# edwinyosorahardjo/compressjs-flattened

Hardware: AMD Instinct MI355X
Metric: bzip2 -9 compress MB/s at 1/2/4/8 MI355X; bit-exact output size vs ref (higher is better)
Workload: dtype u32; 1 GPU; Bzip2.compressFile level 9 (899981-byte blocks) on 1 x 100000000 bytes enwik8-shaped synthetic text (tools/textgen.c seed 1), device-resident; per_gpu_bytes=100000000, level=9, parallelism=1 GPU

## Files before the change

### compressjs-flattened_amd/csrc/ctx.h

```cpp
#pragma once
#include "cjs_internal.h"
#include "rle1.h"
#include "mtf.h"
#include "huff.h"

namespace cjs {
struct BatchWork;
void batch_destroy(BatchWork* b);
struct BatchDelete { void operator()(BatchWork* b) const { batch_destroy(b); } };
}

struct cjs_ctx {
  int device = 0, level = 0;
  uint32_t cap = 0;
  size_t max_input = 0, max_blocks = 0, range_blocks = 0;
  cjs::Arena arena;
  cjs::Rle1Work rle;
  cjs::BwtWork bwt;
  cjs::MtfWork mtf;
  cjs::HuffWork huff;
  uint8_t* d_blocks = nullptr;
  uint8_t* d_U = nullptr;
  uint32_t* d_pidx = nullptr;
  cjs::Owner<cjs::BatchWork*, cjs::BatchDelete> batch;
  cjs::Pinned<uint64_t> h_scalars;
  cjs::Stream stream;
  cjs::Stream side;
  cjs::Event ev_join, ev_fork;
  cjs::Stream tail;
  cjs::Event ev_tail, ev_piece[8];
  cjs::EventTimer timer;
  uint32_t sh_nb = 0, sh_first = 0, sh_cnt = 0, sh_state = 0;
  bool stage_times = true;
};

namespace cjs {
int blocks_through_tables(cjs_ctx* c, const uint8_t* d_in, size_t n, uint32_t nb, uint32_t last_len, uint32_t f, uint32_t cnt, cjs_stats* st, bool stage_times);
}
```

### compressjs-flattened_amd/csrc/mtf.h

```cpp
#pragma once
#include "cjs_internal.h"

namespace cjs {

struct MtfBufs {
  uint32_t* hpos;
  uint8_t* hsym;
  uint8_t* hrank;
  uint8_t* lists;
  uint16_t* A;
  uint32_t* freq;
  uint8_t* alist;
  uint32_t *asz, *nheads, *npos;
  int* segkeys;
  size_t seg_stride;
  size_t list_stride, a_stride, hstride;
};

struct MtfWork {
  size_t max_blocks = 0;
  uint32_t stride = 0;
  MtfBufs b{};
  static size_t list_stride_for(uint32_t stride) { return ((size_t)(stride + 255) / 256 + 1) * 256; }
  static size_t seg_stride_for(uint32_t stride) { return ((size_t)stride + 8191) / 8192 + 1; }
  static size_t hstride_for(uint32_t stride) { return ((size_t)stride + 15) & ~(size_t)15; }
  static size_t a_stride_for(uint32_t stride) { return ((size_t)stride + 2 + 7) & ~(size_t)7; }
  static size_t bytes_needed(size_t max_blocks, uint32_t stride);
  int carve(Arena& a, size_t max_blocks, uint32_t stride);
  MtfWork view(size_t first, size_t count) const {
    MtfWork v = *this;
    v.max_blocks = count;
    v.b.hpos += first * b.hstride; v.b.hsym += first * b.hstride; v.b.hrank += first * b.hstride;
    v.b.lists += first * b.list_stride; v.b.A += first * b.a_stride; v.b.freq += first * 258; v.b.alist += first * 256;
    v.b.asz += first; v.b.nheads += first; v.b.npos += first;
    v.b.segkeys += first * b.seg_stride * 256;
    return v;
  }
};

int mtf_run(hipStream_t s, MtfWork& w, const uint8_t* d_U, uint32_t nb, const uint32_t* d_blen);

}
```

### compressjs-flattened_amd/csrc/mtf.hip

```cpp
#include "cjs_internal.h"
#include "prims.hpp"
#include "mtf.h"

namespace cjs {

#ifndef CJS_MTF_CHUNK
#define CJS_MTF_CHUNK 512
#endif
#ifndef CJS_MTF_CL_THREADS
#define CJS_MTF_CL_THREADS 256
#endif
constexpr int MTF_CHUNK = CJS_MTF_CHUNK;
constexpr int MTF_CL_THREADS = CJS_MTF_CL_THREADS;

constexpr uint32_t MT_TILE = 4096;
constexpr uint32_t HT_PER = 16, HT_TILE = 1024 * HT_PER;
__device__ __forceinline__ uint32_t head_flags4(const uint8_t* __restrict__ u, bool row0, uint32_t p0, uint32_t n, uint32_t& mine) {
  mine = 0;
  if (p0 >= n) return 0u;
  const uintptr_t a = (uintptr_t)(u + p0);
  const uint32_t* al = reinterpret_cast<const uint32_t*>(a & ~(uintptr_t)3);
  const uint32_t sh = (uint32_t)(a & 3);
  const bool first = row0 && p0 == 0;
  const uint32_t wm = first ? 0u : al[-1], w0 = al[0], w1 = sh ? al[1] : 0u;
  mine = __builtin_amdgcn_alignbyte(w1, w0, sh);
  uint32_t prev = __builtin_amdgcn_alignbyte(w0, wm, sh) >> 24;
  uint32_t fm = 0;
#pragma unroll
  for (int j = 0; j < 4; j++) {
    const uint32_t p = p0 + j, c = (mine >> (8 * j)) & 0xFFu;
    if (p < n && (p == 0 || c != prev)) fm |= 1u << j;
    prev = c;
  }
  return fm;
}
__global__ __launch_bounds__(1024) void mtf_head_count(const uint8_t* __restrict__ U, uint32_t stride, const uint32_t* __restrict__ blen,
                                                       uint32_t* __restrict__ tcnt, uint32_t tpb, uint32_t* __restrict__ uflag) {
  __shared__ uint32_t used[256];
  __shared__ uint32_t sm[16];
  const uint32_t blk = blockIdx.y, tile = blockIdx.x, n = blen[blk];
  const uint32_t base = tile * HT_TILE;
  if (base >= n) { if (threadIdx.x == 0) tcnt[(size_t)blk * tpb + tile] = 0; return; }
  const uint8_t* u = U + (size_t)blk * stride;
  if (threadIdx.x < 256) used[threadIdx.x] = 0;
  __syncthreads();
  const uint32_t p0 = base + threadIdx.x * HT_PER;
  uint32_t m4[4] = {0, 0, 0, 0};
  uint32_t prev = 0, cnt = 0;
  if (p0 < n) {
    const uintptr_t a = (uintptr_t)(u + p0);
    const uint32_t* al = reinterpret_cast<const uint32_t*>(a & ~(uintptr_t)3);
    const uint32_t sh = (uint32_t)(a & 3);
    const bool first = blk == 0 && p0 == 0;
    const uint32_t wm = first ? 0u : al[-1], w0 = al[0], w1 = al[1], w2 = al[2], w3 = al[3], w4 = sh ? al[4] : 0u;
    m4[0] = __builtin_amdgcn_alignbyte(w1, w0, sh); m4[1] = __builtin_amdgcn_alignbyte(w2, w1, sh);
    m4[2] = __builtin_amdgcn_alignbyte(w3, w2, sh); m4[3] = __builtin_amdgcn_alignbyte(w4, w3, sh);
    prev = __builtin_amdgcn_alignbyte(w0, wm, sh) >> 24;
  }
#pragma unroll
  for (int j = 0; j < (int)HT_PER; j++) {
    const uint32_t p = p0 + j;
    const uint32_t c = p < n ? (m4[j >> 2] >> (8 * (j & 3))) & 0xFFu : 0u;
    if (p < n && (p == 0 || c != prev)) { cnt++; used[c] = 1; }
    prev = c;
  }
  const uint32_t tot = block_sum<1024>(cnt, sm);
  if (threadIdx.x == 0) tcnt[(size_t)blk * tpb + tile] = tot;
  if (threadIdx.x < 256 && used[threadIdx.x]) uflag[(size_t)blk * 258 + threadIdx.x] = 1;
}
__global__ __launch_bounds__(1024) void mtf_head_write(const uint8_t* __restrict__ U, uint32_t stride, const uint32_t* __restrict__ blen,
                                                       MtfBufs mb, const uint32_t* __restrict__ tcnt, uint32_t tpb) {
  __shared__ uint32_t sm[16];
  const uint32_t blk = blockIdx.y, tile = blockIdx.x, n = blen[blk];
  const uint32_t base = tile * HT_TILE;
  if (base >= n) return;
  const uint8_t* u = U + (size_t)blk * stride;
  uint32_t* hpos = mb.hpos + (size_t)blk * mb.hstride;
  uint8_t* hsym = mb.hsym + (size_t)blk * mb.hstride;
  uint32_t run = tcnt[(size_t)blk * tpb + tile];
  for (uint32_t r = 0; r < HT_TILE / 4096u; r++) {
    const uint32_t p0 = base + r * 4096u + threadIdx.x * 4u;
    if (base + r * 4096u >= n) break;
    uint32_t mine;
    const uint32_t fm = head_flags4(u, blk == 0, p0, n, mine);
    uint32_t tot;
    uint32_t o = run + block_excl_sum<1024>((uint32_t)__builtin_popcount(fm), sm, tot);
#pragma unroll
    for (int j = 0; j < 4; j++) if ((fm >> j) & 1u) { hpos[o] = p0 + j; hsym[o] = (uint8_t)(mine >> (8 * j)); o++; }
    run += tot;
  }
}
__global__ __launch_bounds__(1024) void mtf_head_scan(MtfBufs mb, uint32_t* __restrict__ tcnt, uint32_t tpb, const uint32_t* __restrict__ uflag) {
  __shared__ uint32_t sm[16];
  const uint32_t blk = blockIdx.x;
  uint32_t tot;
  const uint32_t v = threadIdx.x < tpb ? tcnt[(size_t)blk * tpb + threadIdx.x] : 0u;
  const uint32_t ex = block_excl_sum<1024>(v, sm, tot);
  if (threadIdx.x < tpb) tcnt[(size_t)blk * tpb + threadIdx.x] = ex;
  if (threadIdx.x == 0) mb.nheads[blk] = tot;
  const uint32_t f = threadIdx.x < 256 ? uflag[(size_t)blk * 258 + threadIdx.x] : 0u;
  uint32_t asz;
  const uint32_t ax = block_excl_sum<1024>(f, sm, asz);
  if (f) mb.alist[(size_t)blk * 256 + ax] = (uint8_t)threadIdx.x;
  if (threadIdx.x == 0) mb.asz[blk] = asz;
}

constexpr int MTF_SEG = 32;
__global__ __launch_bounds__(256) void mtf_seg_last(MtfBufs mb) {
  __shared__ int last[4][256];
  const uint32_t blk = blockIdx.y, seg = blockIdx.x, H = mb.nheads[blk];
  const uint32_t h0 = seg * MTF_SEG * MTF_CHUNK;
  if (h0 >= H) return;
  const uint32_t h1 = h0 + MTF_SEG * MTF_CHUNK < H ? h0 + MTF_SEG * MTF_CHUNK : H;
  const uint8_t* hsym = mb.hsym + (size_t)blk * mb.hstride;
#pragma unroll
  for (int r = 0; r < 4; r++) last[r][threadIdx.x] = -1;
  __syncthreads();
  int* mine = last[threadIdx.x & 3];
  for (uint32_t h = h0 + threadIdx.x; h < h1; h += 256) atomicMax(&mine[hsym[h]], (int)h);
  __syncthreads();
  const int a01 = last[0][threadIdx.x] > last[1][threadIdx.x] ? last[0][threadIdx.x] : last[1][threadIdx.x];
  const int a23 = last[2][threadIdx.x] > last[3][threadIdx.x] ? last[2][threadIdx.x] : last[3][threadIdx.x];
  mb.segkeys[((size_t)blk * mb.seg_stride + seg) * 256 + threadIdx.x] = a01 > a23 ? a01 : a23;
}
__global__ __launch_bounds__(256) void mtf_seg_scan(MtfBufs mb) {
  __shared__ uint32_t used[256];
  const uint32_t blk = blockIdx.x, H = mb.nheads[blk], asz = mb.asz[blk];
  const uint32_t nseg = (H + MTF_SEG * MTF_CHUNK - 1) / (MTF_SEG * MTF_CHUNK);
  used[threadIdx.x] = 0;
  __syncthreads();
  if (threadIdx.x < asz) used[mb.alist[(size_t)blk * 256 + threadIdx.x]] = 1;
  __syncthreads();
  const int d = threadIdx.x;
  int key = used[d] ? 255 - d : -1000;
  int* sk = mb.segkeys + (size_t)blk * mb.seg_stride * 256;
  for (uint32_t sgi = 0; sgi < nseg; sgi++) {
    const int l = sk[(size_t)sgi * 256 + d];
    sk[(size_t)sgi * 256 + d] = key;
    if (l >= 0) key = 256 + l;
  }
}
__global__ __launch_bounds__(MTF_CL_THREADS) void mtf_chunk_lists(MtfBufs mb) {
  __shared__ int keys[256];
  __shared__ uint8_t symof[256];
  __shared__ uint8_t uof[256];
  __shared__ uint32_t part[4][256];
  const uint32_t blk = blockIdx.y, seg = blockIdx.x, H = mb.nheads[blk], nu = mb.asz[blk];
  const uint32_t nch = (H + MTF_CHUNK - 1) / MTF_CHUNK;
  const uint32_t c0 = seg * MTF_SEG;
  if (c0 >= nch) return;
  const uint32_t c1 = c0 + MTF_SEG < nch ? c0 + MTF_SEG : nch;
  const uint8_t* hsym = mb.hsym + (size_t)blk * mb.hstride;
  uint8_t* lists = mb.lists + (size_t)blk * mb.list_stride;
  if (threadIdx.x < nu) {
    const uint8_t sym = mb.alist[(size_t)blk * 256 + threadIdx.x];
    symof[threadIdx.x] = sym; uof[sym] = (uint8_t)threadIdx.x;
    keys[threadIdx.x] = mb.segkeys[((size_t)blk * mb.seg_stride + seg) * 256 + sym];
  }
  __syncthreads();
  constexpr uint32_t NQ = MTF_CL_THREADS / 256;
  const uint32_t d = threadIdx.x & 255u, q = threadIdx.x >> 8, per = (nu + NQ - 1u) / NQ;
  const uint32_t j0 = q * per < nu ? q * per : nu, j1 = j0 + per < nu ? j0 + per : nu;
  for (uint32_t c = c0; c < c1; c++) {
    if (d < nu) {
      const int kd = keys[d];
      uint32_t cnt = 0;
      for (uint32_t j = j0; j < j1; j++) cnt += keys[j] > kd;
      part[q][d] = cnt;
    }
    __syncthreads();
    if (threadIdx.x < nu) {
      uint32_t p = 0;
#pragma unroll
      for (uint32_t qq = 0; qq < NQ; qq++) p += part[qq][d];
      lists[(size_t)c * 256 + p] = symof[d];
    }
    __syncthreads();
    for (uint32_t i = threadIdx.x; i < MTF_CHUNK; i += MTF_CL_THREADS) {
      const uint32_t h = c * MTF_CHUNK + i;
      if (h < H) atomicMax(&keys[uof[hsym[h]]], (int)(256 + h));
    }
    __syncthreads();
  }
}

constexpr int LROW = 260;
constexpr int MTF_RW = 16;
constexpr uint32_t MTF_NR = 4 * MTF_RW;
#ifndef CJS_MTF_TIERS
#define CJS_MTF_TIERS 0, 4, 8, 10, 12, 14, 16
#endif
constexpr int MTF_NTIER = 6;
__device__ constexpr int MTF_TIER[MTF_NTIER + 1] = {CJS_MTF_TIERS};
__device__ __forceinline__ uint32_t zero_bytes(uint32_t v) { return (v - 0x01010101u) & ~v & 0x80808080u; }
__device__ __forceinline__ uint32_t umin(uint32_t a, uint32_t b) { return a < b ? a : b; }
__device__ __forceinline__ uint32_t first_bit_or_ones(uint32_t z) {
  uint32_t f;
  asm("v_ffbl_b32 %0, %1" : "=v"(f) : "v"(z));
  return f;
}
template <int K> __device__ __forceinline__ uint32_t spread_bit(uint32_t v) {
  uint32_t f;
  asm("v_bfe_i32 %0, %1, %2, 1" : "=v"(f) : "v"(v), "n"(K));
  return f;
}
template <int K, int K1> __device__ __forceinline__ uint32_t mtf_search_words(const uint32_t (&l)[MTF_RW], uint32_t bc, uint32_t m) {
  if constexpr (K < K1) {
    const uint32_t ka = first_bit_or_ones(zero_bytes(l[K] ^ bc)) | (32u * K);
    const uint32_t kb = first_bit_or_ones(zero_bytes(l[K + 1] ^ bc)) | (32u * (K + 1));
    return mtf_search_words<K + 2, K1>(l, bc, umin(m, umin(ka, kb)));
  } else {
    return m;
  }
}
template <int T> __device__ __forceinline__ uint32_t mtf_search_tier(const uint32_t (&l)[MTF_RW], uint32_t bc, uint32_t m) {
  return mtf_search_words<MTF_TIER[T], MTF_TIER[T + 1]>(l, bc, m);
}
template <int K, int K0> __device__ __forceinline__ void mtf_shift_words(uint32_t (&l)[MTF_RW], uint32_t bc, uint32_t above, uint32_t g1, uint32_t pm) {
  if constexpr (K >= K0) {
    const uint32_t g = spread_bit<K>(above);
    const uint32_t sh = __builtin_amdgcn_alignbyte(l[K], K ? l[K ? K - 1 : 0] : bc, 3);
    const uint32_t mk = ~g1 | (~g & pm);
    l[K] = (sh & mk) | (l[K] & ~mk);
    mtf_shift_words<K - 1, K0>(l, bc, above, g, pm);
  }
}
template <int T> __device__ __forceinline__ void mtf_shift_tier(uint32_t (&l)[MTF_RW], uint32_t bc, uint32_t above, uint32_t pm) {
  mtf_shift_words<MTF_TIER[T + 1] - 1, MTF_TIER[T]>(l, bc, above, spread_bit<MTF_TIER[T + 1]>(above), pm);
}
__global__ __launch_bounds__(256) void mtf_replay(uint32_t stride, MtfBufs mb) {
  __shared__ uint8_t L[256 * LROW];
  const uint32_t blk = blockIdx.y, H = mb.nheads[blk], asz = mb.asz[blk];
  const uint32_t nch = (H + MTF_CHUNK - 1) / MTF_CHUNK;
  const uint32_t c = blockIdx.x * 256 + threadIdx.x;
  if (blockIdx.x * 256 >= nch) return;
  if (c >= nch) return;
  const uint8_t* hsym = mb.hsym + (size_t)blk * mb.hstride;
  uint8_t* hrank = mb.hrank + (size_t)blk * mb.hstride;
  const uint8_t* lst = mb.lists + (size_t)blk * mb.list_stride + (size_t)c * 256;
  uint8_t* my = L + threadIdx.x * LROW;
  uint32_t l[MTF_RW];
#pragma unroll
  for (int k = 0; k < MTF_RW; k += 4) {
    const uint4 f = *reinterpret_cast<const uint4*>(lst + 4 * k);
    l[k] = f.x; l[k + 1] = f.y; l[k + 2] = f.z; l[k + 3] = f.w;
  }
  for (uint32_t j = MTF_NR; j < asz; j++) my[j] = lst[j];
  const uint32_t h0 = c * MTF_CHUNK, h1 = h0 + MTF_CHUNK < H ? h0 + MTF_CHUNK : H;
  uint4 sv_next = *reinterpret_cast<const uint4*>(hsym + h0);
  for (uint32_t hb = h0; hb < h1; hb += 16) {
    const uint4 sv = sv_next;
    if (hb + 16 < h1) sv_next = *reinterpret_cast<const uint4*>(hsym + hb + 16);
    uint32_t sw[4] = {sv.x, sv.y, sv.z, sv.w}, rw[4] = {0, 0, 0, 0};
    if (hb + 16 > h1) {
      const uint32_t nv = h1 - hb;
#pragma unroll
      for (int q = 1; q < 16; q++)
        if ((uint32_t)q >= nv) {
          const uint32_t p = (sw[(q - 1) >> 2] >> (8 * ((q - 1) & 3))) & 0xFFu;
          sw[q >> 2] = (sw[q >> 2] & ~(0xFFu << (8 * (q & 3)))) | (p << (8 * (q & 3)));
        }
    }
#pragma unroll
    for (int q = 0; q < 16; q++) {
      const uint32_t bc = __builtin_amdgcn_perm(0u, sw[q >> 2], 0x01010101u * (uint32_t)(q & 3));
      uint32_t m = mtf_search_tier<0>(l, bc, ~0u);
      int tier = 0;
      bool more = __any(m == ~0u);
      if (more) { m = mtf_search_tier<1>(l, bc, m); tier = 1; more = __any(m == ~0u); }
      if (more) { m = mtf_search_tier<2>(l, bc, m); tier = 2; more = __any(m == ~0u); }
      if (more) { m = mtf_search_tier<3>(l, bc, m); tier = 3; more = __any(m == ~0u); }
      if (more) { m = mtf_search_tier<4>(l, bc, m); tier = 4; more = __any(m == ~0u); }
      if (more) { m = mtf_search_tier<5>(l, bc, m); tier = 5; }
      uint32_t r = m >> 3;
      if (m == ~0u) {
        const uint8_t s8 = (uint8_t)bc;
        uint8_t prev = (uint8_t)(l[MTF_RW - 1] >> 24);
        for (r = MTF_NR; r < asz; r++) {
          const uint8_t x = my[r];
          my[r] = prev;
          prev = x;
          if (x == s8) break;
        }
      }
      const uint32_t me = umin(m, 8u * MTF_NR - 1u);
      const uint32_t above = 0xFFFFFFFEu << (me >> 5);
      const uint32_t pm = 0xFFFFFFFFu >> (~me & 31u);
      if (tier >= 5) mtf_shift_tier<5>(l, bc, above, pm);
      if (tier >= 4) mtf_shift_tier<4>(l, bc, above, pm);
      if (tier >= 3) mtf_shift_tier<3>(l, bc, above, pm);
      if (tier >= 2) mtf_shift_tier<2>(l, bc, above, pm);
      if (tier >= 1) mtf_shift_tier<1>(l, bc, above, pm);
      mtf_shift_tier<0>(l, bc, above, pm);
      rw[q >> 2] |= r << (8 * (q & 3));
    }
    *reinterpret_cast<uint4*>(hrank + hb) = make_uint4(rw[0], rw[1], rw[2], rw[3]);
  }
}

constexpr uint32_t ET_TILE = 4 * MT_TILE;
__device__ __forceinline__ uint32_t emit_heads4(const uint32_t* __restrict__ hpos, const uint8_t* __restrict__ hrank, uint32_t h0, uint32_t H, uint32_t n,
                                                uint32_t (&lit)[4], uint32_t (&z)[4], uint32_t (&nd)[4], uint32_t (&rk)[4]) {
  uint32_t rk4 = 0, hp[5] = {0, 0, 0, 0, 0}, cnt = 0;
  if (h0 < H) {
    rk4 = *reinterpret_cast<const uint32_t*>(hrank + h0);
    const uint4 p4 = *reinterpret_cast<const uint4*>(hpos + h0);
    hp[0] = p4.x; hp[1] = p4.y; hp[2] = p4.z; hp[3] = p4.w;
    hp[4] = h0 + 4 < H ? hpos[h0 + 4] : n;
  }
#pragma unroll
  for (int j = 0; j < 4; j++) {
    const uint32_t h = h0 + j;
    lit[j] = z[j] = nd[j] = rk[j] = 0;
    if (h < H) {
      const uint32_t r = (rk4 >> (8 * j)) & 0xFFu;
      const uint32_t len = (h + 1 < H ? hp[j + 1] : n) - hp[j];
      lit[j] = r != 0;
      rk[j] = r;
      z[j] = len - lit[j];
      nd[j] = z[j] ? 31u - (uint32_t)__builtin_clz(z[j] + 1u) : 0u;
      cnt += lit[j] + nd[j];
    }
  }
  return cnt;
}
__global__ __launch_bounds__(1024) void mtf_emit_count(const uint32_t* __restrict__ blen, MtfBufs mb, uint32_t* __restrict__ tcnt, uint32_t tpb) {
  __shared__ uint32_t sm[16];
  const uint32_t blk = blockIdx.y, tile = blockIdx.x, n = blen[blk], H = mb.nheads[blk];
  const uint32_t base = tile * ET_TILE;
  if (base >= H) { if (threadIdx.x == 0) tcnt[(size_t)blk * tpb + tile] = 0; return; }
  const uint32_t* hpos = mb.hpos + (size_t)blk * mb.hstride;
  const uint8_t* hrank = mb.hrank + (size_t)blk * mb.hstride;
  uint32_t cnt = 0;
#pragma unroll
  for (uint32_t q = 0; q < 4; q++) {
    uint32_t lit[4], z[4], nd[4], rk[4];
    cnt += emit_heads4(hpos, hrank, base + q * MT_TILE + threadIdx.x * 4u, H, n, lit, z, nd, rk);
  }
  cnt = block_sum<1024>(cnt, sm);
  if (threadIdx.x == 0) tcnt[(size_t)blk * tpb + tile] = cnt;
}
__global__ __launch_bounds__(1024) void mtf_emit_write(const uint32_t* __restrict__ blen, MtfBufs mb, const uint32_t* __restrict__ tcnt, uint32_t tpb) {
  __shared__ uint32_t freq[8 * 258];
  __shared__ uint32_t sm[16];
  const uint32_t blk = blockIdx.y, tile = blockIdx.x, n = blen[blk], H = mb.nheads[blk];
  const uint32_t base = tile * ET_TILE;
  if (base >= H) return;
  const uint32_t* hpos = mb.hpos + (size_t)blk * mb.hstride;
  const uint8_t* hrank = mb.hrank + (size_t)blk * mb.hstride;
  for (int i = threadIdx.x; i < 8 * 258; i += 1024) freq[i] = 0;
  __syncthreads();
  uint16_t* A = mb.A + (size_t)blk * mb.a_stride;
  uint32_t* rep = freq + (threadIdx.x & 7u) * 258u;
  uint32_t n1 = 0, n0 = 0;
  uint32_t run = tcnt[(size_t)blk * tpb + tile];
  for (uint32_t r = 0; r < ET_TILE / MT_TILE && base + r * MT_TILE < H; r++) {
    uint32_t lit[4], z[4], nd[4], rk[4];
    const uint32_t cnt = emit_heads4(hpos, hrank, base + r * MT_TILE + threadIdx.x * 4u, H, n, lit, z, nd, rk);
    uint32_t tot;
    uint32_t o = run + block_excl_sum<1024>(cnt, sm, tot);
#pragma unroll
    for (int j = 0; j < 4; j++) {
      if (lit[j]) { A[o++] = (uint16_t)(rk[j] + 1); atomicAdd(&rep[rk[j] + 1], 1u); }
      const uint32_t v = z[j] + 1u;
      uint32_t nb1 = 0;
      for (uint32_t i = 0; i < nd[j]; i++) { const uint32_t bit = (v >> i) & 1u; A[o++] = (uint16_t)bit; nb1 += bit; }
      n1 += nb1; n0 += nd[j] - nb1;
    }
    run += tot;
  }
  n1 = wave_sum(n1); n0 = wave_sum(n0);
  if (lane_id() == 0) { if (n1) atomicAdd(&freq[1], n1); if (n0) atomicAdd(&freq[0], n0); }
  __syncthreads();
  for (uint32_t i = threadIdx.x; i < 258; i += 1024) {
    uint32_t f = 0;
#pragma unroll
    for (int r = 0; r < 8; r++) f += freq[r * 258 + i];
    if (f) atomicAdd(&mb.freq[(size_t)blk * 258 + i], f);
  }
}
__global__ __launch_bounds__(1024) void mtf_emit_scan(MtfBufs mb, uint32_t* __restrict__ tcnt, uint32_t tpb) {
  __shared__ uint32_t sm[16];
  const uint32_t blk = blockIdx.x, asz = mb.asz[blk];
  uint32_t tot;
  const uint32_t v = threadIdx.x < tpb ? tcnt[(size_t)blk * tpb + threadIdx.x] : 0u;
  const uint32_t ex = block_excl_sum<1024>(v, sm, tot);
  if (threadIdx.x < tpb) tcnt[(size_t)blk * tpb + threadIdx.x] = ex;
  if (threadIdx.x == 0) {
    mb.A[(size_t)blk * mb.a_stride + tot] = (uint16_t)(asz + 1);
    mb.freq[(size_t)blk * 258 + asz + 1] = 1;
    mb.npos[blk] = tot + 1;
  }
}

size_t MtfWork::bytes_needed(size_t max_blocks, uint32_t stride) {
  size_t b = 0;
  auto add = [&](size_t n) { b += (n + 255) & ~(size_t)255; };
  const size_t ls = list_stride_for(stride), as = a_stride_for(stride), hs = hstride_for(stride);
  add(max_blocks * hs * 4); add(max_blocks * hs); add(max_blocks * hs); add(max_blocks * ls);
  add(max_blocks * as * 2); add(max_blocks * 258 * 4); add(max_blocks * 256);
  add(max_blocks * 4); add(max_blocks * 4); add(max_blocks * 4);
  add(max_blocks * seg_stride_for(stride) * 256 * 4);
  return b + 4096;
}
int MtfWork::carve(Arena& a, size_t max_blocks_, uint32_t stride_) {
  max_blocks = max_blocks_; stride = stride_;
  b.list_stride = list_stride_for(stride); b.a_stride = a_stride_for(stride); b.hstride = hstride_for(stride);
  b.hpos = a.take<uint32_t>(max_blocks * b.hstride); b.hsym = a.take<uint8_t>(max_blocks * b.hstride); b.hrank = a.take<uint8_t>(max_blocks * b.hstride);
  b.lists = a.take<uint8_t>(max_blocks * b.list_stride);
  b.A = a.take<uint16_t>(max_blocks * b.a_stride); b.freq = a.take<uint32_t>(max_blocks * 258); b.alist = a.take<uint8_t>(max_blocks * 256);
  b.asz = a.take<uint32_t>(max_blocks); b.nheads = a.take<uint32_t>(max_blocks); b.npos = a.take<uint32_t>(max_blocks);
  b.seg_stride = seg_stride_for(stride);
  b.segkeys = a.take<int>(max_blocks * b.seg_stride * 256);
  return b.segkeys ? 0 : CJS_E_OUT_OF_MEMORY;
}

int mtf_run(hipStream_t s, MtfWork& w, const uint8_t* d_U, uint32_t nb, const uint32_t* d_blen) {
  if (nb == 0) return 0;
  if (nb > w.max_blocks) return CJS_E_INVALID_ARG;
  const uint32_t max_chunks = (w.stride + MTF_CHUNK - 1) / MTF_CHUNK;
  const uint32_t tpb = (w.stride + MT_TILE - 1) / MT_TILE;
  if (tpb > 1024 || (size_t)tpb > (size_t)w.b.seg_stride * 256) return CJS_E_INVALID_ARG;
  uint32_t* tcnt = reinterpret_cast<uint32_t*>(w.b.segkeys);
  dev_fill(s, w.b.freq, 0, (size_t)nb * 258 * 4);
  const uint32_t tph = (w.stride + HT_TILE - 1) / HT_TILE;
  hipLaunchKernelGGL(mtf_head_count, dim3(tph, nb), dim3(1024), 0, s, d_U, w.stride, d_blen, tcnt, tph, w.b.freq);
  hipLaunchKernelGGL(mtf_head_scan, dim3(nb), dim3(1024), 0, s, w.b, tcnt, tph, w.b.freq);
  hipLaunchKernelGGL(mtf_head_write, dim3(tph, nb), dim3(1024), 0, s, d_U, w.stride, d_blen, w.b, tcnt, tph);
  const uint32_t max_segs = (max_chunks + MTF_SEG - 1) / MTF_SEG;
  hipLaunchKernelGGL(mtf_seg_last, dim3(max_segs, nb), dim3(256), 0, s, w.b);
  hipLaunchKernelGGL(mtf_seg_scan, dim3(nb), dim3(256), 0, s, w.b);
  hipLaunchKernelGGL(mtf_chunk_lists, dim3(max_segs, nb), dim3(MTF_CL_THREADS), 0, s, w.b);
  hipLaunchKernelGGL(mtf_replay, dim3((max_chunks + 255) / 256, nb), dim3(256), 0, s, w.stride, w.b);
  dev_fill(s, w.b.freq, 0, (size_t)nb * 258 * 4);
  const uint32_t tpe = (w.stride + ET_TILE - 1) / ET_TILE;
  hipLaunchKernelGGL(mtf_emit_count, dim3(tpe, nb), dim3(1024), 0, s, d_blen, w.b, tcnt, tpe);
  hipLaunchKernelGGL(mtf_emit_scan, dim3(nb), dim3(1024), 0, s, w.b, tcnt, tpe);
  hipLaunchKernelGGL(mtf_emit_write, dim3(tpe, nb), dim3(1024), 0, s, d_blen, w.b, tcnt, tpe);
  CJS_HIP_TRY(hipGetLastError());
  return 0;
}

}
```

### compressjs-flattened_amd/csrc/pipeline.hip

```cpp
#include "cjs_internal.h"
#include "rle1.h"
#include "mtf.h"
#include "huff.h"
#include "ctx.h"
#include "host.h"
#include <stdlib.h>
#include <string.h>
#include <algorithm>
#include <new>
#include <chrono>
#include <condition_variable>
#include <memory>
#include <mutex>
#include <vector>

using namespace cjs;


extern "C" int cjs_ctx_create(cjs_ctx** out, int device, size_t max_input, int level) {
  return cjs_ctx_create_sharded(out, device, max_input, 0, level);
}

extern "C" int cjs_ctx_create_sharded(cjs_ctx** out, int device, size_t max_input, long max_range_blocks, int level) {
  CJS_GUARD_BEGIN
  if (!out) return CJS_E_INVALID_ARG;
  *out = nullptr;
  if (level < 1 || level > 9) return CJS_E_BAD_LEVEL;
  int ndev = 0;
  if (hipGetDeviceCount(&ndev) != hipSuccess || ndev <= 0) return CJS_E_NO_DEVICE;
  if (device < 0) { if (hipGetDevice(&device) != hipSuccess) return CJS_E_NO_DEVICE; }
  if (device >= ndev) return CJS_E_INVALID_ARG;
  CJS_HIP_TRY(hipSetDevice(device));
  std::unique_ptr<cjs_ctx> c(new (std::nothrow) cjs_ctx());
  if (!c) return CJS_E_OUT_OF_MEMORY;
  c->device = device; c->level = level; c->cap = (uint32_t)level * 100000u - 19u;
  if (max_input == 0) max_input = 1;
  c->max_input = max_input;
  c->max_blocks = Rle1Work::max_blocks_for(max_input, c->cap);
  c->range_blocks = (max_range_blocks > 0 && (size_t)max_range_blocks < c->max_blocks) ? (size_t)max_range_blocks : c->max_blocks;
  const size_t rb = c->range_blocks;
  const size_t elems = rb * c->cap;
  size_t bytes = Rle1Work::bytes_needed(max_input, c->cap, rb) + BwtWork::bytes_needed(elems) +
                 MtfWork::bytes_needed(rb, c->cap) + HuffWork::bytes_needed(rb, c->cap) +
                 2 * (elems + 512) + 4 * rb + 65536;
  CJS_TRY(c->arena.init(bytes));
  CJS_TRY(c->rle.carve(c->arena, max_input, c->cap, rb));
  CJS_TRY(c->bwt.carve(c->arena, elems));
  CJS_TRY(c->mtf.carve(c->arena, rb, c->cap));
  CJS_TRY(c->huff.carve(c->arena, rb, c->cap));
  c->d_blocks = c->arena.take<uint8_t>(elems);
  c->d_U = c->arena.take<uint8_t>(elems);
  c->d_pidx = c->arena.take<uint32_t>(rb);
  if (!c->d_pidx) return CJS_E_OUT_OF_MEMORY;
  CJS_HIP_TRY(hipStreamCreate(c->stream.put()));
  CJS_HIP_TRY(hipStreamCreateWithFlags(c->side.put(), hipStreamNonBlocking));
  CJS_HIP_TRY(hipStreamCreateWithFlags(c->tail.put(), hipStreamNonBlocking));
  for (auto& e : c->ev_piece) CJS_HIP_TRY(hipEventCreateWithFlags(e.put(), hipEventDisableTiming));
  CJS_HIP_TRY(hipEventCreateWithFlags(c->ev_tail.put(), hipEventDisableTiming));
  CJS_HIP_TRY(hipEventCreateWithFlags(c->ev_fork.put(), hipEventDisableTiming));
  CJS_HIP_TRY(hipEventCreateWithFlags(c->ev_join.put(), hipEventDisableTiming));
  CJS_HIP_TRY(hipHostMalloc((void**)c->h_scalars.put(), 256));
  CJS_TRY(c->timer.init(c->stream));
  *out = c.release();
  return 0;
  CJS_GUARD_END(CJS_E_OUT_OF_MEMORY, CJS_E_HIP)
}

extern "C" void cjs_ctx_set_stage_times(cjs_ctx* c, int on) { if (c) c->stage_times = on != 0; }

extern "C" void cjs_ctx_destroy(cjs_ctx* c) {
  if (!c) return;
  (void)hipSetDevice(c->device);
  delete c;
}

static int ensure(DevCache& hc, size_t n, int level, long range_blocks, size_t in_bytes, size_t out_bytes) {
  const cjs_ctx* c = hc.ctx;
  if (!c || c->level != level || c->max_input < n || (range_blocks ? c->range_blocks != (size_t)range_blocks : c->range_blocks != c->max_blocks)) {
    cjs_ctx_destroy(hc.ctx); hc.ctx = nullptr;
    CJS_TRY(cjs_ctx_create_sharded(&hc.ctx, -1, n, range_blocks, level));
  }
  if (in_bytes) CJS_TRY(DevCache::grow(hc.d_in, hc.in_cap, in_bytes));
  if (out_bytes) CJS_TRY(DevCache::grow(hc.d_out, hc.out_cap, out_bytes));
  return 0;
}

static int drain_on_error(cjs_ctx* c, int rc) {
  if (rc && c)
    for (hipStream_t s : {c->side.p, c->tail.p, c->stream.p}) if (s) (void)hipStreamSynchronize(s);
  return rc;
}
static int compress_core_impl(cjs_ctx* c, const uint8_t* d_in, size_t n, int level, long first, long count, bool framed,
                              uint8_t* d_out, size_t out_cap, uint64_t* out_bits, uint32_t* block_crcs, long crc_cap,
                              long* total_blocks, cjs_stats* st);
static int compress_core(cjs_ctx* c, const uint8_t* d_in, size_t n, int level, long first, long count, bool framed,
                         uint8_t* d_out, size_t out_cap, uint64_t* out_bits, uint32_t* block_crcs, long crc_cap,
                         long* total_blocks, cjs_stats* st) {
  CJS_GUARD_BEGIN
  return drain_on_error(c, compress_core_impl(c, d_in, n, level, first, count, framed, d_out, out_cap, out_bits, block_crcs, crc_cap, total_blocks, st));
  CJS_GUARD_END(CJS_E_OUT_OF_MEMORY, CJS_E_HIP)
}
int cjs::blocks_through_tables(cjs_ctx* c, const uint8_t* d_in, size_t n, uint32_t nb, uint32_t last_len, uint32_t f, uint32_t cnt, cjs_stats* st, bool stage_times) {
  hipStream_t s = c->stream;
  if (cnt > c->range_blocks) return CJS_E_INVALID_ARG;
  uint32_t n_last = c->cap;
  if (cnt && f + cnt == nb) n_last = last_len;
  CJS_TRY(rle1_finish(s, c->rle, d_in, n, f, cnt, c->d_blocks, c->side, c->ev_fork, c->ev_join));
  if (stage_times) { CJS_HIP_TRY(hipStreamSynchronize(s)); st->ms_rle1 = c->timer.stop(); }
  const uint32_t pieces = (stage_times || !c->tail || (uint64_t)cnt * c->cap < 400000000ull) ? 1u : 4u;
  if (cnt && pieces == 1) {
    if (stage_times) c->timer.start();
    CJS_TRY(bwt_run(s, c->bwt, c->d_blocks, cnt, c->cap, n_last, true, c->d_U, c->d_pidx, st, stage_times));
    if (stage_times) { st->ms_bwt = c->timer.stop(); c->timer.start(); }
    CJS_TRY(mtf_run(s, c->mtf, c->d_U, cnt, c->rle.block_len + f));
    if (stage_times) { CJS_HIP_TRY(hipStreamSynchronize(s)); st->ms_mtf = c->timer.stop(); c->timer.start(); }
    CJS_TRY(huff_tables_run(s, c->huff, cnt, c->mtf.b.A, c->mtf.b.a_stride, c->mtf.b.npos, c->mtf.b.asz, c->mtf.b.freq, c->mtf.b.alist));
    if (stage_times) { CJS_HIP_TRY(hipStreamSynchronize(s)); st->ms_huff = c->timer.stop(); }
  } else if (cnt) {
    const uint32_t per = (cnt + pieces - 1) / pieces;
    LaunchTimes keep;
    for (uint32_t i = 0, k0 = 0; k0 < cnt; i++, k0 += per) {
      const uint32_t kc = std::min(per, cnt - k0);
      const bool has_last = k0 + kc == cnt;
      CJS_TRY(bwt_run(s, c->bwt, c->d_blocks + (size_t)k0 * c->cap, kc, c->cap, has_last ? n_last : c->cap, true, c->d_U + (size_t)k0 * c->cap, c->d_pidx + k0, st, false));
      if (st) { c->bwt.lt.move_into(keep); }
      CJS_HIP_TRY(hipEventRecord(c->ev_piece[i], s));
      CJS_HIP_TRY(hipStreamWaitEvent(c->tail, c->ev_piece[i], 0));
      MtfWork mv = c->mtf.view(k0, kc);
      HuffWork hv = c->huff.view(k0, kc);
      CJS_TRY(mtf_run(c->tail, mv, c->d_U + (size_t)k0 * c->cap, kc, c->rle.block_len + f + k0));
      CJS_TRY(huff_tables_run(c->tail, hv, kc, mv.b.A, mv.b.a_stride, mv.b.npos, mv.b.asz, mv.b.freq, mv.b.alist));
    }
    if (st) keep.move_into(c->bwt.lt);
    CJS_HIP_TRY(hipEventRecord(c->ev_tail, c->tail));
    CJS_HIP_TRY(hipStreamWaitEvent(s, c->ev_tail, 0));
  }
  return 0;
}
static int compress_core_impl(cjs_ctx* c, const uint8_t* d_in, size_t n, int level, long first, long count, bool framed,
                              uint8_t* d_out, size_t out_cap, uint64_t* out_bits, uint32_t* block_crcs, long crc_cap,
                              long* total_blocks, cjs_stats* st) {
  if (!c || level != c->level) return CJS_E_INVALID_ARG;
  if (n > c->max_input) return CJS_E_INVALID_ARG;
  if (((uintptr_t)d_out & 3) != 0) return CJS_E_INVALID_ARG;
  CJS_HIP_TRY(hipSetDevice(c->device));
  hipStream_t s = c->stream;
  c->sh_state = 0;
  EventTimer whole;
  const bool stage_times = st && c->stage_times;
  if (st) { memset(st, 0, sizeof *st); CJS_TRY(whole.init(s)); whole.start(); }
  uint32_t nb = 0, last_len = 0;
  if (stage_times) c->timer.start();
  CJS_TRY(rle1_run(s, c->rle, d_in, n, &nb, &last_len));
  if (total_blocks) *total_blocks = (long)nb;
  if (first < 0 || first > (long)nb) return CJS_E_INVALID_ARG;
  if (count < 0 || first + count > (long)nb) count = (long)nb - first;
  const uint32_t f = (uint32_t)first, cnt = (uint32_t)count;
  CJS_TRY(blocks_through_tables(c, d_in, n, nb, last_len, f, cnt, st, stage_times));
  if (stage_times) c->timer.start();
  if (cnt && n && c->side) CJS_HIP_TRY(hipStreamWaitEvent(s, c->ev_join, 0));
  const uint64_t start_bit = framed ? 32 : 0;
  CJS_TRY(huff_pack_run(s, c->huff, nb, f, cnt, start_bit, level, framed ? 1 : 0, framed ? 1 : 0, c->mtf.b.A, c->mtf.b.a_stride,
                        c->mtf.b.npos, c->mtf.b.asz, c->mtf.b.alist, c->rle.block_crc, c->d_pidx, (uint32_t*)d_out, out_cap & ~(size_t)3));
  CJS_HIP_TRY(hipMemcpyAsync(c->h_scalars, c->huff.scalars, 24, hipMemcpyDeviceToHost, s));
  if (block_crcs && nb) {
    if ((long)nb > crc_cap) return CJS_E_OUTPUT_TOO_SMALL;
    CJS_HIP_TRY(hipMemcpyAsync(block_crcs, c->rle.block_crc, 4 * (size_t)nb, hipMemcpyDeviceToHost, s));
  }
  CJS_HIP_TRY(hipStreamSynchronize(s));
  if (c->h_scalars[2]) return CJS_E_OUTPUT_TOO_SMALL;
  *out_bits = c->h_scalars[0];
  if (st) {
    if (stage_times) st->ms_pack = c->timer.stop();
    if (!stage_times && cnt) c->bwt.lt.resolve(st);
    st->ms_total = whole.stop();
    st->blocks = cnt; st->bytes_in = n; st->bytes_out = (*out_bits + 7) / 8;
  }
  return 0;
}

extern "C" size_t cjs_bzip2_shard_share_bytes(size_t n, int world) {
  if (world < 1) return 0;
  return Rle1Work::share_bytes(Rle1Work::tiles_per_rank(n, (uint32_t)world));
}
extern "C" int cjs_bzip2_shard_tiles(cjs_ctx* c, const uint8_t* d_in, size_t n, int rank, int world, void* d_share) {
  CJS_GUARD_BEGIN
  if (!c || !d_share || world < 1 || rank < 0 || rank >= world || n > c->max_input) return CJS_E_INVALID_ARG;
  CJS_HIP_TRY(hipSetDevice(c->device));
  c->sh_state = 0;
  const uint32_t tpr = Rle1Work::tiles_per_rank(n, (uint32_t)world);
  const uint64_t t0 = (uint64_t)rank * tpr, Tn = Rle1Work::tiles_for(n);
  if (t0 < Tn) CJS_TRY(rle1_tiles(c->stream, c->rle, d_in, n, (uint32_t)t0, (uint32_t)std::min<uint64_t>(Tn, t0 + tpr), (uint8_t*)d_share, tpr));
  CJS_HIP_TRY(hipStreamSynchronize(c->stream));
  c->sh_state = 1;
  return 0;
  CJS_GUARD_END(CJS_E_OUT_OF_MEMORY, CJS_E_HIP)
}
__global__ void shard_meta_kernel(const uint32_t* __restrict__ bitlen, const uint32_t* __restrict__ block_crc, uint32_t first, uint32_t cnt, uint64_t* __restrict__ out) {
  if (threadIdx.x || blockIdx.x) return;
  uint64_t bits = 0; uint32_t c = 0;
  for (uint32_t k = 0; k < cnt; k++) { bits += bitlen[k]; c = ((c << 1) | (c >> 31)) ^ block_crc[first + k]; }
  out[0] = bits; out[1] = c;
}
static void shard_range(uint32_t total, int rank, int world, uint32_t& first, uint32_t& count) {
  const uint32_t share = total ? (total + (uint32_t)world - 1u) / (uint32_t)world : 0u;
  first = std::min<uint64_t>((uint64_t)rank * share, total);
  count = std::min<uint32_t>(share, total - first);
}
static int shard_blocks_impl(cjs_ctx* c, const uint8_t* d_in, size_t n, int level, int rank, int world, const void* d_shares, cjs_shard_meta* meta, cjs_stats* st) {
  if (!c || !meta || level != c->level || world < 1 || rank < 0 || rank >= world || n > c->max_input || (world > 1 && !d_shares)) return CJS_E_INVALID_ARG;
  if (c->sh_state != 1 && d_shares) return CJS_E_INVALID_ARG;
  CJS_HIP_TRY(hipSetDevice(c->device));
  hipStream_t s = c->stream;
  c->sh_state = 0;
  EventTimer whole;
  const bool stage_times = st && c->stage_times;
  if (st) { memset(st, 0, sizeof *st); CJS_TRY(whole.init(s)); whole.start(); }
  if (stage_times) c->timer.start();
  uint32_t nb = 0, last_len = 0;
  if (d_shares) CJS_TRY(rle1_tables_from_shares(s, c->rle, n, (const uint8_t*)d_shares, Rle1Work::tiles_per_rank(n, (uint32_t)world)));
  else if (n) CJS_TRY(rle1_tiles(s, c->rle, d_in, n, 0u, Rle1Work::tiles_for(n), nullptr, 0u));
  CJS_TRY(rle1_walk_run(s, c->rle, d_in, n, &nb, &last_len));
  uint32_t f = 0, cnt = 0;
  shard_range(nb, rank, world, f, cnt);
  CJS_TRY(blocks_through_tables(c, d_in, n, nb, last_len, f, cnt, st, stage_times));
  if (cnt && n && c->side) CJS_HIP_TRY(hipStreamWaitEvent(s, c->ev_join, 0));
  hipLaunchKernelGGL(shard_meta_kernel, dim3(1), dim3(1), 0, s, c->huff.b.bitlen, c->rle.block_crc, f, cnt, c->huff.scalars + 4);
  CJS_HIP_TRY(hipMemcpyAsync(c->h_scalars + 4, c->huff.scalars + 4, 16, hipMemcpyDeviceToHost, s));
  CJS_HIP_TRY(hipStreamSynchronize(s));
  meta->bits = c->h_scalars[4]; meta->crc_fold = (uint32_t)c->h_scalars[5];
  meta->total_blocks = nb; meta->first_block = f; meta->blocks = cnt;
  c->sh_nb = nb; c->sh_first = f; c->sh_cnt = cnt; c->sh_state = 2;
  if (st) {
    if (!stage_times && cnt) c->bwt.lt.resolve(st);
    st->ms_total = whole.stop(); st->blocks = cnt; st->bytes_in = n; st->bytes_out = (meta->bits + 7) / 8;
  }
  return 0;
}
extern "C" int cjs_bzip2_shard_blocks(cjs_ctx* c, const uint8_t* d_in, size_t n, int level, int rank, int world, const void* d_shares,
                                      cjs_shard_meta* meta, cjs_stats* stats) {
  CJS_GUARD_BEGIN
  return drain_on_error(c, shard_blocks_impl(c, d_in, n, level, rank, world, d_shares, meta, stats));
  CJS_GUARD_END(CJS_E_OUT_OF_MEMORY, CJS_E_HIP)
}
static int shard_pack_core(cjs_ctx* c, int level, bool header, bool trailer, uint64_t start, uint64_t bits, uint32_t scrc, uint8_t* d_out, size_t out_cap,
                           size_t* frag_off, size_t* frag_len, uint64_t* stream_off) {
  hipStream_t s = c->stream;
  const uint64_t local_start = header ? 32 : (start & 31), end_local = local_start + bits;
  const PackShard ps{scrc, trailer ? 0 : 1};
  CJS_TRY(huff_pack_run(s, c->huff, c->sh_nb, c->sh_first, c->sh_cnt, local_start, level, header ? 1 : 0, trailer ? 1 : 0, c->mtf.b.A, c->mtf.b.a_stride,
                        c->mtf.b.npos, c->mtf.b.asz, c->mtf.b.alist, c->rle.block_crc, c->d_pidx, (uint32_t*)d_out, out_cap & ~(size_t)3, &ps));
  CJS_HIP_TRY(hipMemcpyAsync(c->h_scalars, c->huff.scalars, 24, hipMemcpyDeviceToHost, s));
  CJS_HIP_TRY(hipStreamSynchronize(s));
  if (c->h_scalars[2]) return CJS_E_OUTPUT_TOO_SMALL;
  const uint64_t word0 = header ? 0 : (start >> 5);
  const uint64_t skip = (!header && (start & 31)) ? 4 : 0;
  const uint64_t end_bytes = trailer ? (end_local + 80 + 7) / 8 : ((end_local + 31) / 32) * 4;
  *frag_off = (size_t)skip; *frag_len = (size_t)(end_bytes > skip ? end_bytes - skip : 0); *stream_off = word0 * 4 + skip;
  return 0;
}
static void shard_layout(const cjs_shard_meta* metas, int world, int rank, uint64_t& start, uint64_t& total, uint32_t& scrc, int& writer) {
  start = 32; total = 32; scrc = 0; writer = 0;
  for (int r = 0; r < world; r++) {
    if (r < rank) start += metas[r].bits;
    total += metas[r].bits;
    const uint32_t rot = metas[r].blocks & 31u;
    scrc = (rot ? ((scrc << rot) | (scrc >> (32 - rot))) : scrc) ^ metas[r].crc_fold;
// ... 443 lines not shown
```

Baseline: 9175 MB/s.

## Rewrite MTF chunk-list kernel as single-wave ballot scan and overlap emit-count on side stream

The per-chunk MTF list builder now runs as one 64-lane wave. It places the symbols seen in each chunk at the front using ballot/mbcnt prefix counts instead of an O(nu^2) key-comparison rank per chunk. The emit count and scan kernels now derive literal flags from head positions instead of ranks, so they can run on a side stream in parallel with chunk_lists and replay, joined before emit_write. This adds a dedicated etcnt buffer and fork/join events. The risks are low occupancy from the 64-thread blocks and extra stream synchronization.

```diff
diff --git a/compressjs-flattened_amd/csrc/ctx.h b/compressjs-flattened_amd/csrc/ctx.h
--- a/compressjs-flattened_amd/csrc/ctx.h
+++ b/compressjs-flattened_amd/csrc/ctx.h
@@ -27,6 +27,7 @@
   cjs::Stream stream;
   cjs::Stream side;
   cjs::Event ev_join, ev_fork;
+  cjs::Event ev_mtf_fork, ev_mtf_join;
   cjs::Stream tail;
   cjs::Event ev_tail, ev_piece[8];
   cjs::EventTimer timer;
diff --git a/compressjs-flattened_amd/csrc/mtf.h b/compressjs-flattened_amd/csrc/mtf.h
--- a/compressjs-flattened_amd/csrc/mtf.h
+++ b/compressjs-flattened_amd/csrc/mtf.h
@@ -14,6 +14,8 @@
   uint32_t *asz, *nheads, *npos;
   int* segkeys;
   size_t seg_stride;
+  uint32_t* etcnt;
+  size_t et_stride;
   size_t list_stride, a_stride, hstride;
 };
 
@@ -23,6 +25,7 @@
   MtfBufs b{};
   static size_t list_stride_for(uint32_t stride) { return ((size_t)(stride + 255) / 256 + 1) * 256; }
   static size_t seg_stride_for(uint32_t stride) { return ((size_t)stride + 8191) / 8192 + 1; }
+  static size_t et_stride_for(uint32_t stride) { return ((size_t)stride + 16383) / 16384; }
   static size_t hstride_for(uint32_t stride) { return ((size_t)stride + 15) & ~(size_t)15; }
   static size_t a_stride_for(uint32_t stride) { return ((size_t)stride + 2 + 7) & ~(size_t)7; }
   static size_t bytes_needed(size_t max_blocks, uint32_t stride);
@@ -34,10 +37,12 @@
     v.b.lists += first * b.list_stride; v.b.A += first * b.a_stride; v.b.freq += first * 258; v.b.alist += first * 256;
     v.b.asz += first; v.b.nheads += first; v.b.npos += first;
     v.b.segkeys += first * b.seg_stride * 256;
+    v.b.etcnt += first * b.et_stride;
     return v;
   }
 };
 
-int mtf_run(hipStream_t s, MtfWork& w, const uint8_t* d_U, uint32_t nb, const uint32_t* d_blen);
+int mtf_run(hipStream_t s, MtfWork& w, const uint8_t* d_U, uint32_t nb, const uint32_t* d_blen,
+            hipStream_t side = nullptr, hipEvent_t ev_fork = nullptr, hipEvent_t ev_join = nullptr);
 
 }
diff --git a/compressjs-flattened_amd/csrc/mtf.hip b/compressjs-flattened_amd/csrc/mtf.hip
--- a/compressjs-flattened_amd/csrc/mtf.hip
+++ b/compressjs-flattened_amd/csrc/mtf.hip
@@ -7,11 +7,7 @@
 #ifndef CJS_MTF_CHUNK
 #define CJS_MTF_CHUNK 512
 #endif
-#ifndef CJS_MTF_CL_THREADS
-#define CJS_MTF_CL_THREADS 256
-#endif
 constexpr int MTF_CHUNK = CJS_MTF_CHUNK;
-constexpr int MTF_CL_THREADS = CJS_MTF_CL_THREADS;
 
 constexpr uint32_t MT_TILE = 4096;
 constexpr uint32_t HT_PER = 16, HT_TILE = 1024 * HT_PER;
@@ -140,11 +136,15 @@
     if (l >= 0) key = 256 + l;
   }
 }
-__global__ __launch_bounds__(MTF_CL_THREADS) void mtf_chunk_lists(MtfBufs mb) {
+__device__ __forceinline__ uint32_t lanes_below(uint64_t m, uint32_t acc) {
+  return __builtin_amdgcn_mbcnt_hi((uint32_t)(m >> 32), __builtin_amdgcn_mbcnt_lo((uint32_t)m, acc));
+}
+__global__ __launch_bounds__(64) void mtf_chunk_lists(MtfBufs mb) {
+  static_assert(MTF_CHUNK == 512, "eight heads per lane");
   __shared__ int keys[256];
-  __shared__ uint8_t symof[256];
-  __shared__ uint8_t uof[256];
-  __shared__ uint32_t part[4][256];
+  __shared__ int last[256];
+  __shared__ uint32_t nlw[64 + 16];
+  uint8_t* nl = reinterpret_cast<uint8_t*>(nlw);
   const uint32_t blk = blockIdx.y, seg = blockIdx.x, H = mb.nheads[blk], nu = mb.asz[blk];
   const uint32_t nch = (H + MTF_CHUNK - 1) / MTF_CHUNK;
   const uint32_t c0 = seg * MTF_SEG;
@@ -152,35 +152,85 @@
   const uint32_t c1 = c0 + MTF_SEG < nch ? c0 + MTF_SEG : nch;
   const uint8_t* hsym = mb.hsym + (size_t)blk * mb.hstride;
   uint8_t* lists = mb.lists + (size_t)blk * mb.list_stride;
-  if (threadIdx.x < nu) {
-    const uint8_t sym = mb.alist[(size_t)blk * 256 + threadIdx.x];
-    symof[threadIdx.x] = sym; uof[sym] = (uint8_t)threadIdx.x;
-    keys[threadIdx.x] = mb.segkeys[((size_t)blk * mb.seg_stride + seg) * 256 + sym];
-  }
-  __syncthreads();
-  constexpr uint32_t NQ = MTF_CL_THREADS / 256;
-  const uint32_t d = threadIdx.x & 255u, q = threadIdx.x >> 8, per = (nu + NQ - 1u) / NQ;
-  const uint32_t j0 = q * per < nu ? q * per : nu, j1 = j0 + per < nu ? j0 + per : nu;
+  const uint32_t lane = threadIdx.x;
+  uint32_t sym[4];
+  int kd[4];
+#pragma unroll
+  for (int q = 0; q < 4; q++) {
+    const uint32_t u = lane + 64u * q;
+    sym[q] = 0; kd[q] = 0;
+    if (u < nu) {
+      sym[q] = mb.alist[(size_t)blk * 256 + u];
+      kd[q] = mb.segkeys[((size_t)blk * mb.seg_stride + seg) * 256 + sym[q]];
+      keys[u] = kd[q];
+    }
+    last[u] = -1;
+  }
+  nlw[lane] = 0;
+  __syncthreads();
+  uint32_t cnt[4] = {0, 0, 0, 0};
+#pragma unroll 4
+  for (uint32_t j = 0; j < nu; j++) {
+    const int k = keys[j];
+#pragma unroll
+    for (int q = 0; q < 4; q++) cnt[q] += k > kd[q];
+  }
+#pragma unroll
+  for (int q = 0; q < 4; q++) if (lane + 64u * q < nu) nl[cnt[q]] = (uint8_t)sym[q];
+  __syncthreads();
+  uint32_t lw = nlw[lane];
+  const uint2* hs8 = reinterpret_cast<const uint2*>(hsym) + lane;
+  uint2 sv_next = c0 + 1 < c1 ? hs8[(size_t)c0 * (MTF_CHUNK / 8)] : make_uint2(0u, 0u);
   for (uint32_t c = c0; c < c1; c++) {
-    if (d < nu) {
-      const int kd = keys[d];
-      uint32_t cnt = 0;
-      for (uint32_t j = j0; j < j1; j++) cnt += keys[j] > kd;
-      part[q][d] = cnt;
+    reinterpret_cast<uint32_t*>(lists + (size_t)c * 256)[lane] = lw;
+    if (c + 1 == c1) break;
+    const uint2 sv = sv_next;
+    if (c + 2 < c1) sv_next = hs8[(size_t)(c + 1) * (MTF_CHUNK / 8)];
+    const int base = (int)(c * MTF_CHUNK), h0 = base + 8 * (int)lane;
+    uint32_t s[8];
+#pragma unroll
+    for (int r = 0; r < 8; r++) {
+      s[r] = ((r < 4 ? sv.x : sv.y) >> (8 * (r & 3))) & 0xFFu;
+      atomicMax(&last[s[r]], h0 + r);
     }
     __syncthreads();
-    if (threadIdx.x < nu) {
-      uint32_t p = 0;
-#pragma unroll
-      for (uint32_t qq = 0; qq < NQ; qq++) p += part[qq][d];
-      lists[(size_t)c * 256 + p] = symof[d];
+    int lh[8], ll[4];
+#pragma unroll
+    for (int r = 0; r < 8; r++) lh[r] = last[s[r]];
+#pragma unroll
+    for (int j = 0; j < 4; j++) ll[j] = last[(lw >> (8 * j)) & 0xFFu];
+    uint32_t own = 0, k = 0, below = 0;
+#pragma unroll
+    for (int r = 0; r < 8; r++) {
+      const bool mark = lh[r] == h0 + r;
+      const uint64_t m = __ballot(mark);
+      own |= (uint32_t)mark << r;
+      k += (uint32_t)__builtin_popcountll(m);
+      below = lanes_below(m, below);
+    }
+    const uint32_t spare = 256u + lane;
+    uint32_t o = k - below - (uint32_t)__builtin_popcount(own);
+#pragma unroll
+    for (int r = 7; r >= 0; r--) {
+      const bool mark = (own >> r) & 1u;
+      nl[mark ? o : spare] = (uint8_t)s[r];
+      o += mark;
+    }
+    uint32_t pres = 0, before = 0;
+#pragma unroll
+    for (int j = 0; j < 4; j++) {
+      const bool in = 4u * lane + j < nu && ll[j] >= base;
+      pres |= (uint32_t)in << j;
+      before = lanes_below(__ballot(in), before);
+    }
+#pragma unroll
+    for (int j = 0; j < 4; j++) {
+      const uint32_t p = 4u * lane + j;
+      const bool stays = p < nu && !((pres >> j) & 1u);
+      nl[stays ? k + p - before - (uint32_t)__builtin_popcount(pres & ((1u << j) - 1u)) : spare] = (uint8_t)(lw >> (8 * j));
     }
     __syncthreads();
-    for (uint32_t i = threadIdx.x; i < MTF_CHUNK; i += MTF_CL_THREADS) {
-      const uint32_t h = c * MTF_CHUNK + i;
-      if (h < H) atomicMax(&keys[uof[hsym[h]]], (int)(256 + h));
-    }
-    __syncthreads();
+    lw = nlw[lane];
   }
 }
 
@@ -299,11 +349,13 @@
 }
 
 constexpr uint32_t ET_TILE = 4 * MT_TILE;
-__device__ __forceinline__ uint32_t emit_heads4(const uint32_t* __restrict__ hpos, const uint8_t* __restrict__ hrank, uint32_t h0, uint32_t H, uint32_t n,
+static_assert(ET_TILE == 16384, "MtfWork::et_stride_for");
+template <bool RANKS>
+__device__ __forceinline__ uint32_t emit_heads4(const uint32_t* __restrict__ hpos, const uint8_t* __restrict__ hrank, uint32_t h0, uint32_t H, uint32_t n, bool lit0,
                                                 uint32_t (&lit)[4], uint32_t (&z)[4], uint32_t (&nd)[4], uint32_t (&rk)[4]) {
   uint32_t rk4 = 0, hp[5] = {0, 0, 0, 0, 0}, cnt = 0;
   if (h0 < H) {
-    rk4 = *reinterpret_cast<const uint32_t*>(hrank + h0);
+    if constexpr (RANKS) rk4 = *reinterpret_cast<const uint32_t*>(hrank + h0);
     const uint4 p4 = *reinterpret_cast<const uint4*>(hpos + h0);
     hp[0] = p4.x; hp[1] = p4.y; hp[2] = p4.z; hp[3] = p4.w;
     hp[4] = h0 + 4 < H ? hpos[h0 + 4] : n;
@@ -315,7 +367,7 @@
     if (h < H) {
       const uint32_t r = (rk4 >> (8 * j)) & 0xFFu;
       const uint32_t len = (h + 1 < H ? hp[j + 1] : n) - hp[j];
-      lit[j] = r != 0;
+      lit[j] = RANKS ? r != 0 : (h != 0 || lit0);
       rk[j] = r;
       z[j] = len - lit[j];
       nd[j] = z[j] ? 31u - (uint32_t)__builtin_clz(z[j] + 1u) : 0u;
@@ -330,12 +382,12 @@
   const uint32_t base = tile * ET_TILE;
   if (base >= H) { if (threadIdx.x == 0) tcnt[(size_t)blk * tpb + tile] = 0; return; }
   const uint32_t* hpos = mb.hpos + (size_t)blk * mb.hstride;
-  const uint8_t* hrank = mb.hrank + (size_t)blk * mb.hstride;
+  const bool lit0 = mb.hsym[(size_t)blk * mb.hstride] != mb.alist[(size_t)blk * 256];
   uint32_t cnt = 0;
 #pragma unroll
   for (uint32_t q = 0; q < 4; q++) {
     uint32_t lit[4], z[4], nd[4], rk[4];
-    cnt += emit_heads4(hpos, hrank, base + q * MT_TILE + threadIdx.x * 4u, H, n, lit, z, nd, rk);
+    cnt += emit_heads4<false>(hpos, nullptr, base + q * MT_TILE + threadIdx.x * 4u, H, n, lit0, lit, z, nd, rk);
   }
   cnt = block_sum<1024>(cnt, sm);
   if (threadIdx.x == 0) tcnt[(size_t)blk * tpb + tile] = cnt;
@@ -356,7 +408,7 @@
   uint32_t run = tcnt[(size_t)blk * tpb + tile];
   for (uint32_t r = 0; r < ET_TILE / MT_TILE && base + r * MT_TILE < H; r++) {
     uint32_t lit[4], z[4], nd[4], rk[4];
-    const uint32_t cnt = emit_heads4(hpos, hrank, base + r * MT_TILE + threadIdx.x * 4u, H, n, lit, z, nd, rk);
+    const uint32_t cnt = emit_heads4<true>(hpos, hrank, base + r * MT_TILE + threadIdx.x * 4u, H, n, false, lit, z, nd, rk);
     uint32_t tot;
     uint32_t o = run + block_excl_sum<1024>(cnt, sm, tot);
 #pragma unroll
@@ -401,6 +453,7 @@
   add(max_blocks * as * 2); add(max_blocks * 258 * 4); add(max_blocks * 256);
   add(max_blocks * 4); add(max_blocks * 4); add(max_blocks * 4);
   add(max_blocks * seg_stride_for(stride) * 256 * 4);
+  add(max_blocks * et_stride_for(stride) * 4);
   return b + 4096;
 }
 int MtfWork::carve(Arena& a, size_t max_blocks_, uint32_t stride_) {
@@ -412,31 +465,40 @@
   b.asz = a.take<uint32_t>(max_blocks); b.nheads = a.take<uint32_t>(max_blocks); b.npos = a.take<uint32_t>(max_blocks);
   b.seg_stride = seg_stride_for(stride);
   b.segkeys = a.take<int>(max_blocks * b.seg_stride * 256);
-  return b.segkeys ? 0 : CJS_E_OUT_OF_MEMORY;
-}
-
-int mtf_run(hipStream_t s, MtfWork& w, const uint8_t* d_U, uint32_t nb, const uint32_t* d_blen) {
+  b.et_stride = et_stride_for(stride);
+  b.etcnt = a.take<uint32_t>(max_blocks * b.et_stride);
+  return b.etcnt ? 0 : CJS_E_OUT_OF_MEMORY;
+}
+
+int mtf_run(hipStream_t s, MtfWork& w, const uint8_t* d_U, uint32_t nb, const uint32_t* d_blen, hipStream_t side, hipEvent_t ev_fork, hipEvent_t ev_join) {
   if (nb == 0) return 0;
   if (nb > w.max_blocks) return CJS_E_INVALID_ARG;
   const uint32_t max_chunks = (w.stride + MTF_CHUNK - 1) / MTF_CHUNK;
-  const uint32_t tpb = (w.stride + MT_TILE - 1) / MT_TILE;
-  if (tpb > 1024 || (size_t)tpb > (size_t)w.b.seg_stride * 256) return CJS_E_INVALID_ARG;
+  const uint32_t tph = (w.stride + HT_TILE - 1) / HT_TILE;
+  const uint32_t tpe = (w.stride + ET_TILE - 1) / ET_TILE;
+  if ((w.stride + MT_TILE - 1) / MT_TILE > 1024 || (size_t)tph > (size_t)w.b.seg_stride * 256 || tpe != w.b.et_stride) return CJS_E_INVALID_ARG;
   uint32_t* tcnt = reinterpret_cast<uint32_t*>(w.b.segkeys);
   dev_fill(s, w.b.freq, 0, (size_t)nb * 258 * 4);
-  const uint32_t tph = (w.stride + HT_TILE - 1) / HT_TILE;
   hipLaunchKernelGGL(mtf_head_count, dim3(tph, nb), dim3(1024), 0, s, d_U, w.stride, d_blen, tcnt, tph, w.b.freq);
   hipLaunchKernelGGL(mtf_head_scan, dim3(nb), dim3(1024), 0, s, w.b, tcnt, tph, w.b.freq);
+  dev_fill(s, w.b.freq, 0, (size_t)nb * 258 * 4);
   hipLaunchKernelGGL(mtf_head_write, dim3(tph, nb), dim3(1024), 0, s, d_U, w.stride, d_blen, w.b, tcnt, tph);
   const uint32_t max_segs = (max_chunks + MTF_SEG - 1) / MTF_SEG;
   hipLaunchKernelGGL(mtf_seg_last, dim3(max_segs, nb), dim3(256), 0, s, w.b);
   hipLaunchKernelGGL(mtf_seg_scan, dim3(nb), dim3(256), 0, s, w.b);
-  hipLaunchKernelGGL(mtf_chunk_lists, dim3(max_segs, nb), dim3(MTF_CL_THREADS), 0, s, w.b);
+  hipStream_t cs = s;
+  if (side) {
+    CJS_HIP_TRY(hipEventRecord(ev_fork, s));
+    CJS_HIP_TRY(hipStreamWaitEvent(side, ev_fork, 0));
+    cs = side;
+  }
+  hipLaunchKernelGGL(mtf_emit_count, dim3(tpe, nb), dim3(1024), 0, cs, d_blen, w.b, w.b.etcnt, tpe);
+  hipLaunchKernelGGL(mtf_emit_scan, dim3(nb), dim3(1024), 0, cs, w.b, w.b.etcnt, tpe);
+  if (side) CJS_HIP_TRY(hipEventRecord(ev_join, side));
+  hipLaunchKernelGGL(mtf_chunk_lists, dim3(max_segs, nb), dim3(64), 0, s, w.b);
   hipLaunchKernelGGL(mtf_replay, dim3((max_chunks + 255) / 256, nb), dim3(256), 0, s, w.stride, w.b);
-  dev_fill(s, w.b.freq, 0, (size_t)nb * 258 * 4);
-  const uint32_t tpe = (w.stride + ET_TILE - 1) / ET_TILE;
-  hipLaunchKernelGGL(mtf_emit_count, dim3(tpe, nb), dim3(1024), 0, s, d_blen, w.b, tcnt, tpe);
-  hipLaunchKernelGGL(mtf_emit_scan, dim3(nb), dim3(1024), 0, s, w.b, tcnt, tpe);
-  hipLaunchKernelGGL(mtf_emit_write, dim3(tpe, nb), dim3(1024), 0, s, d_blen, w.b, tcnt, tpe);
+  if (side) CJS_HIP_TRY(hipStreamWaitEvent(s, ev_join, 0));
+  hipLaunchKernelGGL(mtf_emit_write, dim3(tpe, nb), dim3(1024), 0, s, d_blen, w.b, w.b.etcnt, tpe);
   CJS_HIP_TRY(hipGetLastError());
   return 0;
 }
diff --git a/compressjs-flattened_amd/csrc/pipeline.hip b/compressjs-flattened_amd/csrc/pipeline.hip
--- a/compressjs-flattened_amd/csrc/pipeline.hip
+++ b/compressjs-flattened_amd/csrc/pipeline.hip
@@ -59,6 +59,8 @@
   CJS_HIP_TRY(hipEventCreateWithFlags(c->ev_tail.put(), hipEventDisableTiming));
   CJS_HIP_TRY(hipEventCreateWithFlags(c->ev_fork.put(), hipEventDisableTiming));
   CJS_HIP_TRY(hipEventCreateWithFlags(c->ev_join.put(), hipEventDisableTiming));
+  CJS_HIP_TRY(hipEventCreateWithFlags(c->ev_mtf_fork.put(), hipEventDisableTiming));
+  CJS_HIP_TRY(hipEventCreateWithFlags(c->ev_mtf_join.put(), hipEventDisableTiming));
   CJS_HIP_TRY(hipHostMalloc((void**)c->h_scalars.put(), 256));
   CJS_TRY(c->timer.init(c->stream));
   *out = c.release();
@@ -112,7 +114,7 @@
     if (stage_times) c->timer.start();
     CJS_TRY(bwt_run(s, c->bwt, c->d_blocks, cnt, c->cap, n_last, true, c->d_U, c->d_pidx, st, stage_times));
     if (stage_times) { st->ms_bwt = c->timer.stop(); c->timer.start(); }
-    CJS_TRY(mtf_run(s, c->mtf, c->d_U, cnt, c->rle.block_len + f));
+    CJS_TRY(mtf_run(s, c->mtf, c->d_U, cnt, c->rle.block_len + f, c->side, c->ev_mtf_fork, c->ev_mtf_join));
     if (stage_times) { CJS_HIP_TRY(hipStreamSynchronize(s)); st->ms_mtf = c->timer.stop(); c->timer.start(); }
     CJS_TRY(huff_tables_run(s, c->huff, cnt, c->mtf.b.A, c->mtf.b.a_stride, c->mtf.b.npos, c->mtf.b.asz, c->mtf.b.freq, c->mtf.b.alist));
     if (stage_times) { CJS_HIP_TRY(hipStreamSynchronize(s)); st->ms_huff = c->timer.stop(); }
```

After: 9307 MB/s (median of 6 runs). +1.4%, better.
